# LouisPwr/CarpeDeam

Measured on AMD Instinct MI355X. Metric: corrected bases/sec on 50M×100bp synthetic reads (dhigh), 1/2/4/8 GPU, higher is better.
Workload: dtype u8 (2-bit packed bases; int32 scores; software x87 f80 likelihood sums)

## Files before the change

carpedeam_amd/csrc/aggvote.h:

```cpp
#pragma once
#include "runsort.h"

namespace aggv {

struct Ent { uint32_t id, diag, cs; };
constexpr uint32_t PENDING = 0xFFFFFFFFu;

__global__ __launch_bounds__(1024) void k_seg_flags(const uint32_t *__restrict__ recRep, uint64_t nRec, uint32_t *__restrict__ flag) {
    const uint64_t j = (uint64_t) blockIdx.x * blockDim.x + threadIdx.x;
    if (j <= nRec) flag[j] = (j < nRec && (j == 0 || recRep[j - 1] != recRep[j])) ? 1u : 0u;
}
__global__ __launch_bounds__(1024) void k_seg_fill(const uint32_t *__restrict__ recRep, uint64_t nRec, uint32_t *__restrict__ segOfRec, uint32_t *__restrict__ segRep,
                                                   unsigned long long *__restrict__ segFirstRec, uint32_t *__restrict__ entCnt) {
    const uint64_t j = (uint64_t) blockIdx.x * blockDim.x + threadIdx.x;
    if (j > nRec) return;
    const uint32_t ex = segOfRec[j];
    if (j == nRec) { segFirstRec[ex] = nRec; return; }
    const bool start = j == 0 || recRep[j - 1] != recRep[j];
    const uint32_t g = start ? ex : ex - 1;
    segOfRec[j] = g;
    if (start) { segRep[g] = recRep[j]; segFirstRec[g] = j; entCnt[g] = PENDING; }
}

struct AggArgs {
    const uint64_t *keys; const uint64_t *recVal; const unsigned long long *dst; uint64_t nRec;
    const uint32_t *segOfRec, *segRep; const unsigned long long *segFirstRec; uint64_t nSeg;
    unsigned long long *entOff; uint32_t *entCnt; unsigned long long *perRep;
    Ent *ent; unsigned long long *cursor; unsigned long long cap; unsigned int *overflow;
    int repShift, diagBits; uint32_t idBits;
    uint32_t maxD;
    const uint64_t *sorted;
    const unsigned long long *list; const unsigned int *count;
    bucket::BigList hard;
    unsigned int nextClass = 0;
    int wideWord = 0;
};
constexpr int AG_H = 1024, AG_D = 512, AG_IDX = 9, AG_ORD = 11;
constexpr unsigned long long AG_CHUNK = 2048;
inline unsigned long long aggChunkSlack(unsigned long long units, unsigned long long segments, int cuCount) {
    const unsigned long long g = (unsigned long long) cuCount * 64;
    return (3 * std::min(units + 1, g) + std::min(segments + 1, g)) * AG_CHUNK;
}
static_assert((1 << AG_IDX) >= AG_D && (1 << AG_ORD) > runsort::U_T, "aggregation geometry");
__device__ __forceinline__ uint32_t aggHash(uint64_t k) { return (uint32_t) ((k * 0x9E3779B97F4A7C15ull) >> 40); }

#ifndef CDM_AGG_MINW
#define CDM_AGG_MINW 4
#endif
template <int NT, int ITEMS, typename W = uint64_t>
__global__ __launch_bounds__(NT, CDM_AGG_MINW) void k_unit_agg(AggArgs a) {
    using namespace runsort;
    __shared__ __align__(8) unsigned char sTab[AG_H * 16];
    unsigned long long *tKey = reinterpret_cast<unsigned long long *>(sTab);
    unsigned int *tCnt = reinterpret_cast<unsigned int *>(sTab + AG_H * 8), *tLast = reinterpret_cast<unsigned int *>(sTab + AG_H * 12);
    unsigned int *oFirst = reinterpret_cast<unsigned int *>(sTab), *oEnt = oFirst + (U_T + 2), *oHit = oEnt + (U_T + 2);
    static_assert(3 * (U_T + 2) * 4 <= AG_H * 16, "the directory fits the table's memory");
    __shared__ unsigned long long dKey[AG_D];
    __shared__ unsigned int dCnt[AG_D], dLast[AG_D];
    __shared__ uint16_t sPerm[AG_D];
    __shared__ uint64_t sGStart[NT];
    __shared__ uint32_t sGOff[NT], sGSeg[NT];
    __shared__ unsigned int sDistinct, sOver, sMaxOrd;
    __shared__ unsigned long long sBase, sChunkAt, sChunkEnd;
    const int tid = threadIdx.x, lane = tid & 63, wave = tid >> 6;
    const unsigned int nUnits = *a.count;
    if (tid == 0) { sChunkAt = 0; sChunkEnd = 0; }
    const int lowBits = a.repShift - 1;
    const uint64_t lowMask = (1ull << lowBits) - 1ull;
    for (unsigned int item = blockIdx.x; item < nUnits; item += gridDim.x) {
        const uint64_t base = a.list[3 * (size_t) item];
        const int m = (int) (a.list[3 * (size_t) item + 1] - base);
        const uint64_t rec0 = a.list[3 * (size_t) item + 2];
        const uint32_t g0 = a.segOfRec[rec0];
        for (int i = tid; i < AG_H; i += NT) { tKey[i] = ~0ull; tCnt[i] = 0u; tLast[i] = 0u; }
        if (tid == 0) { sDistinct = 0; sOver = 0; sMaxOrd = 0; }
        __syncthreads();
        const unsigned long long endG = base + (uint64_t) m;
        for (uint64_t c0 = rec0; c0 < a.nRec; c0 += NT) {
            const uint64_t j = c0 + tid;
            const unsigned long long d = j < a.nRec ? a.dst[j] : ~0ull;
            const bool valid = d < endG;
            sGOff[tid] = valid ? (uint32_t) (d - base) : (uint32_t) m;
            sGStart[tid] = valid ? (a.recVal[j] >> RUN_CNT_BITS) : 0ull;
            sGSeg[tid] = valid ? a.segOfRec[j] - g0 : 0u;
            const int nr = __syncthreads_count(valid);
            if (nr == 0) break;
            const int e0 = (int) sGOff[0], e1 = (nr == NT) ? (int) min((unsigned long long) m, (j0Next(a.dst, a.nRec, c0 + NT) - base)) : m;
            if (tid == 0) sMaxOrd = max(sMaxOrd, sGSeg[nr - 1]);
            for (int eb = e0; eb < e1; eb += NT * ITEMS) {
                uint64_t key[ITEMS]; uint32_t ordv[ITEMS];
#pragma unroll
                for (int k = 0; k < ITEMS; k++) {
                    const int e = eb + k * NT + tid;
                    if (e < e1) {
                        int r = 0;
#pragma unroll
                        for (int st = NT / 2; st > 0; st >>= 1) if (r + st < nr && (int) sGOff[r + st] <= e) r += st;
                        key[k] = a.keys[sGStart[r] + (uint64_t) (e - (int) sGOff[r])];
                        ordv[k] = sGSeg[r];
                    }
                }
#pragma unroll
                for (int k = 0; k < ITEMS; k++) {
                    const int e = eb + k * NT + tid;
                    if (e < e1) {
                        const uint64_t hk = ((uint64_t) ordv[k] << lowBits) | ((key[k] >> 1) & lowMask);
                        const unsigned int last = ((unsigned int) e << 1) | (unsigned int) (key[k] & 1ull);
                        uint32_t h = aggHash(hk) & (AG_H - 1);
                        int probe = 0;
                        for (; probe < AG_H; probe++) {
                            unsigned long long old = __hip_atomic_load(&tKey[h], __ATOMIC_RELAXED, __HIP_MEMORY_SCOPE_WORKGROUP);
                            if (old == ~0ull) {
                                old = atomicCAS(&tKey[h], ~0ull, (unsigned long long) hk);
                                if (old == ~0ull) { atomicAdd(&sDistinct, 1u); old = hk; }
                            }
                            if (old == hk) { atomicAdd(&tCnt[h], 1u); atomicMax(&tLast[h], last); break; }
                            h = (h + 1) & (AG_H - 1);
                        }
                        if (probe == AG_H) sOver = 1u;
                    }
                }
            }
            const bool stop = __syncthreads_or(sDistinct > a.maxD || sOver != 0u);
            if (stop || nr < NT) break;
        }
        __syncthreads();
        if (sDistinct > a.maxD || sOver) {
            if (tid == 0) a.hard.add(base, base + (uint64_t) m);
            __syncthreads();
            continue;
        }
        unsigned int c = 0;
        for (int i = tid; i < AG_H; i += NT) c += tKey[i] != ~0ull;
        unsigned int D;
        unsigned int pos = cdm_block_excl_sum<unsigned int>(c, D);
        for (int i = tid; i < AG_H; i += NT) if (tKey[i] != ~0ull) { dKey[pos] = tKey[i]; dCnt[pos] = tCnt[i]; dLast[pos] = tLast[i]; pos++; }
        __syncthreads();
        if (wave == 0) {
            bucket::sortGroup<W>((int) D, lane,
                [&](int i) { return ((W) dKey[i] << AG_IDX) | (W) i; },
                [&](auto &v) {
                    constexpr int R = sizeof(v) / sizeof(v[0]);
#pragma unroll
                    for (int r = 0; r < R; r++) { const int p = lane * R + r; if (p < (int) D) sPerm[p] = (uint16_t) ((uint32_t) v[r] & ((1u << AG_IDX) - 1u)); }
                });
        }
        const unsigned int nOrd = sMaxOrd + 1u;
        for (unsigned int o = tid; o < nOrd; o += NT) { oFirst[o] = 0xFFFFFFFFu; oEnt[o] = 0u; oHit[o] = 0u; }
        if (tid == 0) {
            if (sChunkAt + D > sChunkEnd) { const unsigned long long want = max(AG_CHUNK, (unsigned long long) D); sChunkAt = atomicAdd(a.cursor, want); sChunkEnd = sChunkAt + want; }
            const unsigned long long b = sChunkAt;
            sChunkAt += D;
            if (b + D > a.cap) { atomicExch(a.overflow, 1u); sBase = ~0ull; } else sBase = b;
        }
        __syncthreads();
        const uint64_t idMask = (1ull << a.idBits) - 1ull, diagMask = (1ull << a.diagBits) - 1ull;
        for (unsigned int p = tid; p < D; p += NT) {
            const uint64_t hk = dKey[sPerm[p]], prev = p ? dKey[sPerm[p - 1]] : ~0ull;
            const uint32_t o = (uint32_t) (hk >> lowBits);
            atomicMin(&oFirst[o], p);
            atomicAdd(&oEnt[o], 1u);
            if (p == 0 || (hk >> a.diagBits) != (prev >> a.diagBits)) {
                const uint32_t id = (uint32_t) ((hk >> a.diagBits) & idMask);
                if (id != a.segRep[g0 + o]) atomicAdd(&oHit[o], 1u);
            }
        }
        __syncthreads();
        const unsigned long long b = sBase;
        if (b != ~0ull) {
            for (unsigned int p = tid; p < D; p += NT) {
                const int i = sPerm[p]; const uint64_t hk = dKey[i];
                Ent e; e.id = (uint32_t) ((hk >> a.diagBits) & idMask); e.diag = (uint32_t) (hk & diagMask); e.cs = (dCnt[i] << 1) | (dLast[i] & 1u);
                a.ent[b + p] = e;
            }
            for (unsigned int o = tid; o < nOrd; o += NT) {
                a.entOff[g0 + o] = b + oFirst[o]; a.entCnt[g0 + o] = oEnt[o];
                a.perRep[a.segRep[g0 + o]] = oHit[o];
            }
        }
        __syncthreads();
    }
}

__global__ __launch_bounds__(1024) void k_pending_list(const uint32_t *__restrict__ entCnt, uint64_t nSeg, uint32_t *__restrict__ list, unsigned int *__restrict__ cnt) {
    const uint64_t g = (uint64_t) blockIdx.x * blockDim.x + threadIdx.x;
    const bool p = g < nSeg && entCnt[g] == PENDING;
    const uint32_t q = cdm_block_append(cnt, p);
    if (p) list[q] = (uint32_t) g;
}
__global__ __launch_bounds__(256) void k_rle_segment(AggArgs a, const uint32_t *__restrict__ list, const unsigned int *__restrict__ nList) {
    const unsigned int n = *nList;
    const int lane = threadIdx.x & 63;
    const uint64_t idMask = (1ull << a.idBits) - 1ull, diagMask = (1ull << a.diagBits) - 1ull;
    const uint64_t below = (1ull << lane) - 1ull;
    unsigned long long chunkAt = 0, chunkEnd = 0;
    for (unsigned int it = blockIdx.x * (blockDim.x >> 6) + (threadIdx.x >> 6); it < n; it += gridDim.x * (blockDim.x >> 6)) {
        const uint32_t g = list[it];
        const uint64_t s = a.dst[a.segFirstRec[g]], e = a.dst[a.segFirstRec[g + 1]];
        const uint32_t rep = a.segRep[g];
        unsigned int runs = 0, hits = 0;
        for (uint64_t i = s + lane; i < e; i += 64) {
            const uint64_t k = a.sorted[i], p = i > s ? a.sorted[i - 1] : ~0ull;
            if (i == s || (k >> 1) != (p >> 1)) runs++;
            if (i == s || (k >> (a.diagBits + 1)) != (p >> (a.diagBits + 1))) hits += ((uint32_t) ((k >> (a.diagBits + 1)) & idMask) != rep);
        }
        const unsigned int D = (unsigned int) cdm_wave_sum((int) runs), H = (unsigned int) cdm_wave_sum((int) hits);
        unsigned long long b = 0;
        if (lane == 0) {
            if (chunkAt + D > chunkEnd) { const unsigned long long want = max(AG_CHUNK, (unsigned long long) D); chunkAt = atomicAdd(a.cursor, want); chunkEnd = chunkAt + want; }
            b = chunkAt; chunkAt += D;
            if (b + D > a.cap) { atomicExch(a.overflow, 1u); b = ~0ull; }
            else { a.entOff[g] = b; a.entCnt[g] = D; a.perRep[rep] = H; }
        }
        b = (unsigned long long) __shfl((long long) b, 0, 64);
        if (b == ~0ull) continue;
        unsigned long long run = 0;
        for (uint64_t t0 = s; t0 < e; t0 += 64) {
            const uint64_t i = t0 + lane;
            bool start = false; uint64_t k = 0;
            if (i < e) { k = a.sorted[i]; start = i == s || (k >> 1) != (a.sorted[i - 1] >> 1); }
            const uint64_t m = __ballot(start);
            if (start) {
                const uint64_t later = lane < 63 ? (m >> (lane + 1)) : 0ull;
                uint64_t hi;
                if (later) hi = i + (uint64_t) __ffsll((unsigned long long) later);
                else {
                    uint64_t lo = min(t0 + 63, e - 1); hi = e;
                    while (hi - lo > 1) { const uint64_t mid = lo + ((hi - lo) >> 1); if ((a.sorted[mid] >> 1) == (k >> 1)) lo = mid; else hi = mid; }
                }
                Ent en; en.id = (uint32_t) ((k >> (a.diagBits + 1)) & idMask); en.diag = (uint32_t) ((k >> 1) & diagMask);
                en.cs = ((uint32_t) (hi - i) << 1) | (uint32_t) (a.sorted[hi - 1] & 1ull);
                a.ent[b + run + (unsigned long long) __popcll(m & below)] = en;
            }
            run += (unsigned long long) __popcll(m);
        }
    }
}

struct VoteEntArgs {
    const Ent *ent; const unsigned long long *entOff; const uint32_t *entCnt; const uint32_t *segRep; uint64_t nSeg;
    const uint64_t *hitOff;
    const uint32_t *stale;
    int diagBias;
    const uint32_t *cont = nullptr;
};
constexpr int HEAD_WORDS = 2048;
__global__ void k_head_entries(const Ent *__restrict__ ent, const unsigned long long *__restrict__ entOff, const uint32_t *__restrict__ entCnt, uint64_t nSeg, uint32_t *__restrict__ out) {
    if (nSeg == 0) { out[0] = 0; out[1] = 0; out[2] = 1; out[HEAD_WORDS + 3] = 0; return; }
    const uint32_t id = ent[entOff[0]].id;
    uint32_t words = 0; bool whole = true;
    for (uint64_t g = 0; g < nSeg && whole && words <= (uint32_t) HEAD_WORDS; g++) {
        const Ent *e = ent + entOff[g]; const uint32_t c = entCnt[g];
        for (uint32_t j = 0; j < c; j++) {
            if (e[j].id != id) { whole = false; break; }
            if (words + 2 <= (uint32_t) HEAD_WORDS) { out[3 + words] = e[j].diag | ((e[j].cs & 1u) ? 0u : 1u << 31); out[4 + words] = e[j].cs >> 1; words += 2; }
            else { words = (uint32_t) HEAD_WORDS + 1; whole = false; break; }
        }
    }
    out[0] = words; out[1] = id; out[2] = whole ? 1u : 0u;
    const uint64_t gl = nSeg - 1;
    out[HEAD_WORDS + 3] = ent[entOff[gl] + entCnt[gl] - 1].id;
}
// ... 47 lines not shown
```

carpedeam_amd/csrc/kmermatch.hip:

```cpp
#include <memory>
#include <cstring>

#include "aggvote.h"
#include "kmer_plan.h"
#include "kmer_tuple.h"
#include "kmer_extract.h"
#include "kmer_group.h"
#include "kmer_vote.h"

namespace {

using rx::DoubleBuf;
using namespace kplan;
static_assert(RADIX_BITS == rx::BITS && SLOT_REM_BITS == rx::SLOT_REM, "kmer_plan.h restates the radix sort's geometry");
inline uint64_t deviceBytes() { size_t fr = 0, tot = 0; if (hipMemGetInfo(&fr, &tot) == hipSuccess) return tot; (void) hipGetLastError(); return 0; }
inline Db planDb(const cdm_seqdb *db, int k, bool device = false) { Db d; d.n = db->n; d.maxLen = db->maxLen; d.residues = db->residues; d.k = k; if (device) d.deviceBytes = deviceBytes(); return d; }

struct KmerJobBase {
    virtual ~KmerJobBase() {}
    virtual int phaseA() = 0;
    virtual int staleTail(unsigned long long J) = 0;
    virtual int phaseB(cdm_hits **out) = 0;
    virtual int gatherByRep() = 0;
    virtual int sortFrom(const uint64_t *devKeys, uint64_t nKeys, uint32_t *head, uint64_t info[2]) = 0;
// ... 534 lines not shown
    DoubleBuf<uint32_t> rep; DoubleBuf<uint64_t> val;
};
int recordsByRep(const runsort::RunArgs &ra, bool staged, bool dstIfNone, RepRecords &R, unsigned long long &total) {
    if (staged) { if (int rc = stagedRunRecords(ra, R.r0, R.r1, R.v0, R.v1, R.nRec)) return rc; }
    else if (int rc = runsort::makeRunRecords(s, ra, R.r0, R.r1, R.v0, R.v1, R.nRec)) return rc;
    if (R.nRec == 0 && !dstIfNone) return CDM_OK;
    if (!R.dst.alloc(R.nRec + 1)) { cdm_set_error("cdm_kmermatch: out of device memory (%llu run records)", R.nRec); return CDM_ERR_HIP; }
    if (R.nRec == 0) return CDM_OK;
    R.rep = DoubleBuf<uint32_t>(R.r0.p, R.r1.p); R.val = DoubleBuf<uint64_t>(R.v0.p, R.v1.p);
    if (int rc = rx::sortPairs<uint32_t, uint64_t>(s, ctx->cuCount, R.rep, R.val, (uint64_t) R.nRec, 0, (int) idBits)) return rc;
    hipMemsetAsync(R.val.current() + R.nRec, 0, 8, s);
    if (int rc = cdmscan::exclusiveScanFn<unsigned long long, runsort::RunLen>(s, R.st, runsort::RunLen{R.val.current()}, R.dst.p, (size_t) R.nRec + 1)) return rc;
    hipMemcpyAsync(&total, R.dst.p + R.nRec, 8, hipMemcpyDeviceToHost, s);
    return CDM_OK;
}
int stagedRunRecords(const runsort::RunArgs &whole, DevBuf<uint32_t> &rr0, DevBuf<uint32_t> &rr1, DevBuf<uint64_t> &rv0, DevBuf<uint64_t> &rv1, unsigned long long &nRec) {
    DevBuf<unsigned long long> off; cdmscan::ScanTemp st;
    if (!off.alloc(stagedWaves + 1)) { cdm_set_error("cdm_kmermatch: out of device memory (run records)"); return CDM_ERR_HIP; }
    if (int rc = cdmscan::exclusiveScanFn<unsigned long long, RecCount>(s, st, RecCount{stCnt.p}, off.p, (size_t) stagedWaves + 1)) return rc;
    unsigned long long n1 = 0, n2 = 0;
    hipMemcpyAsync(&n1, off.p + stagedWaves, 8, hipMemcpyDeviceToHost, s);
    DevBuf<uint32_t> q0, q1; DevBuf<uint64_t> w0, w1;
    runsort::RunArgs r2 = whole; r2.keys = whole.keys + kmerSlots; r2.n = whole.n - kmerSlots; r2.skipLo = r2.skipHi = 0; r2.base = kmerSlots;
    if (r2.n) { if (int rc = runsort::makeRunRecords(s, r2, q0, q1, w0, w1, n2)) return rc; }
    if (hipStreamSynchronize(s) != hipSuccess) { cdm_set_error("cdm_kmermatch: run records failed: %s", hipGetErrorString(hipGetLastError())); return CDM_ERR_HIP; }
    unsigned long long nb = nBigRec;
    if (nOvRec) {
        DevBuf<uint64_t> x0, x1; DevBuf<uint32_t> y0, y1;
        const unsigned long long tot = nBigRec + nOvRec;
        if (!x0.alloc(tot) || !x1.alloc(tot) || !y0.alloc(tot) || !y1.alloc(tot)) { cdm_set_error("cdm_kmermatch: out of device memory (run records)"); return CDM_ERR_HIP; }
        if (nBigRec) { hipMemcpyAsync(x0.p, bigRecVal.p, nBigRec * 8, hipMemcpyDeviceToDevice, s); hipMemcpyAsync(y0.p, bigRecRep.p, nBigRec * 4, hipMemcpyDeviceToDevice, s); }
        hipMemcpyAsync(x0.p + nBigRec, ovVal.p, nOvRec * 8, hipMemcpyDeviceToDevice, s); hipMemcpyAsync(y0.p + nBigRec, ovRep.p, nOvRec * 4, hipMemcpyDeviceToDevice, s);
        DoubleBuf<uint64_t> x(x0.p, x1.p); DoubleBuf<uint32_t> y(y0.p, y1.p);
        if (int rc = rx::sortPairs<uint64_t, uint32_t>(s, ctx->cuCount, x, y, (uint64_t) tot, runsort::RUN_CNT_BITS, 64)) return rc;
        bigRecVal.free(); bigRecRep.free();
        bigRecVal.p = x.current() == x0.p ? x0.release() : x1.release(); bigRecRep.p = y.current() == y0.p ? y0.release() : y1.release();
        nb = tot;
    }
    nRec = n1 + nb + n2;
    if (!rr0.alloc(nRec) || !rr1.alloc(nRec) || !rv0.alloc(nRec + 1) || !rv1.alloc(nRec + 1)) { cdm_set_error("cdm_kmermatch: out of device memory (%llu run records)", nRec); return CDM_ERR_HIP; }
    if (n1) hipLaunchKernelGGL(k_rec_compact, CDM_GRID((stagedWaves + REC_WAVES - 1) / REC_WAVES, 256), dim3(256), 0, s, (const uint32_t *) stRep.p, (const uint64_t *) stVal.p, (const unsigned long long *) off.p, (uint64_t) stagedWaves,
                               (uint64_t) stagedOwn, (const uint64_t *) bigRecVal.p, (uint64_t) nb, rr0.p, rv0.p);
    if (nb) hipLaunchKernelGGL(k_rec_place_big, CDM_GRID((nb + 255) / 256, 256), dim3(256), 0, s, (const uint32_t *) bigRecRep.p, (const uint64_t *) bigRecVal.p, (uint64_t) nb, (const uint64_t *) stVal.p, (const uint8_t *) stCnt.p,
                               (const unsigned long long *) off.p, (uint64_t) stagedOwn, rr0.p, rv0.p);
    if (n2) { hipMemcpyAsync(rr0.p + n1 + nb, q0.p, n2 * 4, hipMemcpyDeviceToDevice, s); hipMemcpyAsync(rv0.p + n1 + nb, w0.p, n2 * 8, hipMemcpyDeviceToDevice, s); }
    if (hipStreamSynchronize(s) != hipSuccess) { cdm_set_error("cdm_kmermatch: run records (packing) failed: %s", hipGetErrorString(hipGetLastError())); return CDM_ERR_HIP; }
    if (cdmGetenv("CDM_BUCKET_STATS")) fprintf(stderr, "run records: %llu staged by the grouping kernel, %llu beyond its waves' stages, %llu of its big buckets, %llu of the whole-sequence hash region\n", n1, nOvRec, nBigRec, n2);
    stRep.free(); stVal.free(); stCnt.free(); bigRecRep.free(); bigRecVal.free(); ovRep.free(); ovVal.free(); stagedWaves = 0; nBigRec = 0; nOvRec = 0;
    return CDM_OK;
}
int voteEntries(cdm_hits **out, const uint32_t *contDev = nullptr) {
    DevBuf<unsigned long long> perRepScan;
    if (!perRepScan.alloc((size_t) n + 1)) { cdm_set_error("cdm_kmermatch: out of device memory (vote)"); return CDM_ERR_HIP; }
    cdmscan::ScanTemp st4a;
    if (int rc = cdmscan::exclusiveScan<unsigned long long>(s, st4a, agPerRep.p, perRepScan.p, (size_t) n + 1)) return rc;
    if (int rc = placeHits(perRepScan.p, true, out, [&](cdm_hits *res) {
        aggv::VoteEntArgs va; va.ent = agEnt.p; va.entOff = agEntOff.p; va.entCnt = agEntCnt.p; va.segRep = agSegRep.p; va.nSeg = nSegM; va.hitOff = res->off; va.stale = staleBuf.p; va.diagBias = diagBias; va.cont = contDev;
        if (nSegM) hipLaunchKernelGGL(aggv::k_vote_entries<HitRec>, dim3((unsigned) ((nSegM + 255) / 256)), dim3(256), 0, s, va, res->rec);
    })) return rc;
    agEnt.free(); agEntOff.free(); agEntCnt.free(); agSegRep.free(); agSegOfRec.free(); agSegFirstRec.free(); agPerRep.free(); agPending.free();
    return CDM_OK;
}
template <typename Place>
int placeHits(const unsigned long long *perRepScan, bool sort1R2, cdm_hits **out, Place place) {
    cdm_hits *res = new cdm_hits(); res->n = n;
    if (cdmMalloc(&res->off, ((size_t) n + 1) * 8) != hipSuccess) { delete res; cdm_set_error("cdm_kmermatch: out of device memory"); return CDM_ERR_HIP; }
    hipLaunchKernelGGL(k_offsets, dim3((n + 256) / 256), dim3(256), 0, s, perRepScan, n, res->off);
    uint64_t total = 0;
    hipMemcpyAsync(&total, res->off + n, 8, hipMemcpyDeviceToHost, s);
    { hipError_t e = hipStreamSynchronize(s); if (e != hipSuccess) { cdm_hits_free(res); cdm_set_error("cdm_kmermatch: vote failed: %s", hipGetErrorString(e)); return CDM_ERR_HIP; } }
    res->count = total;
    if (cdmMalloc(&res->rec, (total + 1) * sizeof(HitRec)) != hipSuccess) { cdm_hits_free(res); cdm_set_error("cdm_kmermatch: out of device memory"); return CDM_ERR_HIP; }
    hipLaunchKernelGGL(k_self, dim3((n + 255) / 256), dim3(256), 0, s, res->off, n, res->rec);
    place(res);
    { hipError_t e = hipStreamSynchronize(s); if (e != hipSuccess) { cdm_hits_free(res); cdm_set_error("cdm_kmermatch: placing hits failed: %s", hipGetErrorString(e)); return CDM_ERR_HIP; } }
    float msSort2 = 0; hipEventElapsedTime(&msSort2, ctx->ev0, ctx->ev1);
    ctx->lastMs[2] = msSort1 + msSort2;
    ctx->lastMs[5] = msSort1;
    ctx->lastMs[6] = msSort2;
    if (sort1R2) hipEventElapsedTime(&ctx->lastMs[7], ctx->ev2, ctx->ev3);
    *out = res;
    return CDM_OK;
}
static void aggUnitHook(hipStream_t st, unsigned int grid, const unsigned long long *list, const unsigned int *count, bucket::BigList hard, void *user) {
    aggv::AggArgs *u = reinterpret_cast<aggv::AggArgs *>(user);
    aggv::AggArgs a = *u;
    a.list = list; a.count = count; a.hard = hard;
    const int cls = (int) (u->nextClass++ % runsort::U_CLASSES);
    const unsigned int pad = cdm_lds_pad("CDM_LDS_PAD_AGG");
    if (u->wideWord) {
        if (cls == 0) hipLaunchKernelGGL((aggv::k_unit_agg<256, runsort::U_CLASS_CAP[0] / 256, bucket::u128>), dim3(grid), dim3(256), pad, st, a);
        else if (cls == 1) hipLaunchKernelGGL((aggv::k_unit_agg<256, runsort::U_CLASS_CAP[1] / 256, bucket::u128>), dim3(grid), dim3(256), pad, st, a);
        else hipLaunchKernelGGL((aggv::k_unit_agg<256, runsort::U_CLASS_CAP[2] / 256, bucket::u128>), dim3(grid), dim3(256), pad, st, a);
        return;
    }
    if (cls == 0) hipLaunchKernelGGL((aggv::k_unit_agg<256, runsort::U_CLASS_CAP[0] / 256>), dim3(grid), dim3(256), pad, st, a);
    else if (cls == 1) hipLaunchKernelGGL((aggv::k_unit_agg<256, runsort::U_CLASS_CAP[1] / 256>), dim3(grid), dim3(256), pad, st, a);
    else hipLaunchKernelGGL((aggv::k_unit_agg<256, runsort::U_CLASS_CAP[2] / 256>), dim3(grid), dim3(256), pad, st, a);
}
int aggregate(uint64_t *sortedOut, unsigned long long nGroup, const uint32_t *recRep, const uint64_t *recVal, const unsigned long long *dst, unsigned long long nRec,
              const uint64_t *gk, int top2, unsigned long long capEnt, bool wideWord) {
    using namespace aggv;
    cdmscan::ScanTemp st;
    agEnt.free(); agSegOfRec.free(); agPerRep.free(); agCursor.free(); agFlags.free(); agSegRep.free(); agSegFirstRec.free(); agEntOff.free(); agEntCnt.free(); agPending.free();
    if (!agSegOfRec.alloc(nRec + 2) || !agPerRep.alloc((size_t) n + 1) || !agCursor.alloc(2) || !agFlags.alloc(4)) { cdm_set_error("cdm_kmermatch: out of device memory (aggregation)"); return CDM_ERR_HIP; }
    hipLaunchKernelGGL(k_seg_flags, CDM_GRID((nRec + 1024) / 1024, 1024), dim3(1024), 0, s, recRep, (uint64_t) nRec, agSegOfRec.p);
    if (int rc = cdmscan::exclusiveScan<uint32_t>(s, st, agSegOfRec.p, agSegOfRec.p, (size_t) nRec + 1)) return rc;
    uint32_t nSeg = 0;
    hipMemcpyAsync(&nSeg, agSegOfRec.p + nRec, 4, hipMemcpyDeviceToHost, s);
    if (hipStreamSynchronize(s) != hipSuccess) { cdm_set_error("cdm_kmermatch: aggregation (segments) failed: %s", hipGetErrorString(hipGetLastError())); return CDM_ERR_HIP; }
    if (!agSegRep.alloc(nSeg + 1) || !agSegFirstRec.alloc((size_t) nSeg + 2) || !agEntOff.alloc((size_t) nSeg + 1) || !agEntCnt.alloc((size_t) nSeg + 1) || !agPending.alloc((size_t) nSeg + 1) ||
        !agEnt.alloc(capEnt + 1)) {
        agEnt.free(); cdm_set_error("cdm_kmermatch: out of device memory (aggregation)"); return CDM_ERR_HIP;
    }
    hipLaunchKernelGGL(k_seg_fill, CDM_GRID((nRec + 1024) / 1024, 1024), dim3(1024), 0, s, recRep, (uint64_t) nRec, agSegOfRec.p, agSegRep.p, agSegFirstRec.p, agEntCnt.p);
    hipMemsetAsync(agPerRep.p, 0, ((size_t) n + 1) * 8, s);
    hipMemsetAsync(agCursor.p, 0, 16, s); hipMemsetAsync(agFlags.p, 0, 16, s);
    AggArgs a;
    a.keys = gk; a.recVal = recVal; a.dst = dst; a.nRec = nRec; a.segOfRec = agSegOfRec.p; a.segRep = agSegRep.p; a.segFirstRec = agSegFirstRec.p; a.nSeg = nSeg;
    a.entOff = agEntOff.p; a.entCnt = agEntCnt.p; a.perRep = agPerRep.p; a.ent = agEnt.p; a.cursor = agCursor.p; a.cap = capEnt; a.overflow = agFlags.p;
    a.maxD = AG_D;
    if (const char *e = cdmGetenv("CDM_AGG_D")) { const long v = atol(e); if (v >= 1 && v <= AG_D) a.maxD = (uint32_t) v; }
    a.repShift = (int) (idBits + diagBits + 1); a.diagBits = (int) diagBits; a.idBits = idBits; a.sorted = sortedOut; a.list = nullptr; a.count = nullptr; a.hard.list = nullptr; a.hard.cnt = nullptr;
    a.wideWord = wideWord ? 1 : 0;
    if (runsort::segmentedSortKeys(s, ctx->cuCount, sortedOut, sortedOut, nGroup, (int) (idBits + diagBits + 1), (int) (diagBits + 1), top2, recRep, dst, nRec, gk, recVal, aggUnitHook, &a, wide, agSegOfRec.p, (int) bitsFor((uint64_t) nSeg + 1), agSegFirstRec.p, (uint64_t) nSeg) != CDM_OK) {
        cdm_set_error("cdm_kmermatch: segmented sort 2 failed: %s", hipGetErrorString(hipGetLastError())); return CDM_ERR_HIP;
    }
    hipLaunchKernelGGL(k_pending_list, dim3((unsigned) (((uint64_t) nSeg + 1023) / 1024)), dim3(1024), 0, s, (const uint32_t *) agEntCnt.p, (uint64_t) nSeg, agPending.p, agFlags.p + 1);
    unsigned int fl[4] = {0, 0, 0, 0};
    hipMemcpyAsync(fl, agFlags.p, 16, hipMemcpyDeviceToHost, s);
    if (hipStreamSynchronize(s) != hipSuccess) { cdm_set_error("cdm_kmermatch: aggregation failed: %s", hipGetErrorString(hipGetLastError())); return CDM_ERR_HIP; }
    if (fl[1] && cdmGetenv("CDM_RLE_STATS")) {
        std::vector<uint32_t> pl(fl[1]); std::vector<unsigned long long> fr((size_t) nSeg + 1), dd((size_t) nRec + 1);
        hipMemcpy(pl.data(), agPending.p, (size_t) fl[1] * 4, hipMemcpyDeviceToHost); hipMemcpy(fr.data(), agSegFirstRec.p, ((size_t) nSeg + 1) * 8, hipMemcpyDeviceToHost);
        hipMemcpy(dd.data(), dst, ((size_t) nRec + 1) * 8, hipMemcpyDeviceToHost);
        unsigned long long tot = 0, mx = 0, over4k = 0, over64k = 0, inBig = 0;
        for (uint32_t g : pl) { const unsigned long long m = dd[fr[g + 1]] - dd[fr[g]]; tot += m; mx = std::max(mx, m); if (m > 4096) { over4k++; inBig += m; } if (m > 65536) over64k++; }
        fprintf(stderr, "rle segments: %u of %llu, %llu tuples (longest %llu; %llu beyond 4096 tuples holding %llu, %llu beyond 65536)\n", fl[1], (unsigned long long) nSeg, tot, mx, over4k, inBig, over64k);
    }
    if (fl[1] && !fl[0]) {
        hipLaunchKernelGGL(k_rle_segment, dim3(std::min<unsigned int>((fl[1] + 3) / 4, (unsigned int) ctx->cuCount * 16)), dim3(256), 0, s, a, (const uint32_t *) agPending.p, (const unsigned int *) (agFlags.p + 1));
        hipMemcpyAsync(fl, agFlags.p, 16, hipMemcpyDeviceToHost, s);
        if (hipStreamSynchronize(s) != hipSuccess) { cdm_set_error("cdm_kmermatch: aggregation (segments of the tuple sorters) failed: %s", hipGetErrorString(hipGetLastError())); return CDM_ERR_HIP; }
    }
    unsigned long long used = 0;
    hipMemcpy(&used, agCursor.p, 8, hipMemcpyDeviceToHost);
    if (cdmGetenv("CDM_BUCKET_STATS")) fprintf(stderr, "aggregate: %llu group tuples, %u segments, %llu entries (room for %llu), %u segments through the tuple sorters%s\n", nGroup, nSeg, used, capEnt, fl[1],
                                            fl[0] ? "; entry buffer overflow" : "");
    if (fl[0]) { agEnt.free(); return CDM_ERR_UNSUPPORTED; }
    nSegM = nSeg;
    return CDM_OK;
}
int vote(const uint32_t *contDev, bool ownBuffers, cdm_hits **out) {
    if (haveEntries) return voteEntries(out, contDev);
    const uint64_t *sorted2 = sorted2M; const unsigned long long nGroup = nGroupM;
    DevBuf<unsigned long long> perRep, perRepScan, vTileCnt, vTileOff;
    const uint64_t vTiles = (nGroup + CP_TILE - 1) / CP_TILE;
    if (!perRep.alloc((size_t) n + 1) || !perRepScan.alloc((size_t) n + 1) || !vTileCnt.alloc(vTiles + 1) || !vTileOff.alloc(vTiles + 1)) {
        cdm_set_error("cdm_kmermatch: out of device memory (vote)"); return CDM_ERR_HIP;
    }
    hipMemsetAsync(perRep.p, 0, ((size_t) n + 1) * 8, s);
    hipMemsetAsync(vTileCnt.p, 0, (vTiles + 1) * 8, s);
    VoteArgs va;
    if (ownBuffers && nGroup != nKept) { cdm_set_error("cdm_kmermatch: internal error: %llu group tuples counted, %llu sorted", nKept, nGroup); return CDM_ERR_HIP; }
    va.stale = staleBuf.p; va.cont = contDev;
    va.keys = sorted2; va.n = nGroup; va.idBits = idBits; va.diagBits = diagBits; va.diagBias = diagBias; va.perRep = perRep.p;
    if (nGroup) hipLaunchKernelGGL(k_seg_count, dim3((unsigned) vTiles), dim3(256), 0, s, va, vTileCnt.p);
    cdmscan::ScanTemp st4a, st4b;
    if (int rc = cdmscan::exclusiveScan<unsigned long long>(s, st4a, perRep.p, perRepScan.p, (size_t) n + 1)) return rc;
    if (int rc = cdmscan::exclusiveScan<unsigned long long>(s, st4b, vTileCnt.p, vTileOff.p, (size_t) vTiles + 1)) return rc;
    return placeHits(perRepScan.p, ownBuffers, out, [&](cdm_hits *res) {
        if (nGroup) hipLaunchKernelGGL(k_seg_place, dim3((unsigned) vTiles), dim3(256), cdm_lds_pad("CDM_LDS_PAD_VOTE"), s, va, vTileOff.p, perRepScan.p, res->off, res->rec);
    });
}
int gatherByRep() override {
    using namespace runsort;
    v0.free(); v1.free();
    RunArgs ra; ra.keys = (const uint64_t *) startIo; ra.n = nTuples; ra.skipLo = live; ra.skipHi = kmerSlots; ra.repShift = (int) (idBits + diagBits + 1);
    unsigned long long nOut = 0;
    RepRecords R;
    if (int rc = recordsByRep(ra, stagedWaves != 0, false, R, nOut)) return rc;
    gathered = keys.current();
    if (R.nRec == 0) return CDM_OK;
    hipLaunchKernelGGL(k_run_gather, CDM_GRID((R.nRec + 255) / 256, 256), dim3(256), 0, s, (const uint64_t *) startIo, (const uint64_t *) R.val.current(), (const unsigned long long *) R.dst.p, (uint64_t) R.nRec, gathered);
    if (hipStreamSynchronize(s) != hipSuccess) { cdm_set_error("cdm_kmermatch: gather by representative failed: %s", hipGetErrorString(hipGetLastError())); return CDM_ERR_HIP; }
    if (nOut != nKept) { cdm_set_error("cdm_kmermatch: internal error: %llu group tuples counted, %llu gathered", nKept, nOut); return CDM_ERR_HIP; }
    return CDM_OK;
}
int sortFrom(const uint64_t *devKeys, uint64_t nKeys, uint32_t *head, uint64_t info[2]) override {
    k0.free(); k1.free(); v0.free(); v1.free();
    if (!recvA.alloc(nKeys) || !recvB.alloc(nKeys) || !contBuf.alloc(CONT_CAP + 4)) { cdm_set_error("cdm_kmermatch: out of device memory for %llu received group tuples", (unsigned long long) nKeys); return CDM_ERR_HIP; }
    if (nKeys) hipMemcpyAsync(recvB.p, devKeys, nKeys * 8, hipMemcpyDeviceToDevice, s);
    if (int rc = sort2(recvB.p, nKeys, 0, 0, recvA.p, recvB.p, false)) return rc;
    if (haveEntries) {
        static_assert(aggv::HEAD_WORDS == CONT_CAP, "the words of a head");
        uint32_t lastId = 0;
        hipLaunchKernelGGL(aggv::k_head_entries, dim3(1), dim3(1), 0, s, (const aggv::Ent *) agEnt.p, (const unsigned long long *) agEntOff.p, (const uint32_t *) agEntCnt.p, (uint64_t) nSegM, contBuf.p);
        hipMemcpyAsync(head, contBuf.p, (CONT_CAP + 3) * 4, hipMemcpyDeviceToHost, s);
        hipMemcpyAsync(&lastId, contBuf.p + CONT_CAP + 3, 4, hipMemcpyDeviceToHost, s);
        if (hipStreamSynchronize(s) != hipSuccess) { cdm_set_error("cdm_kmermatch: second half (aggregation) failed: %s", hipGetErrorString(hipGetLastError())); return CDM_ERR_HIP; }
        info[0] = nGroupM; info[1] = lastId;
        return CDM_OK;
    }
    hipLaunchKernelGGL(k_head_segment, dim3(1), dim3(1), 0, s, sorted2M, (uint64_t) nGroupM, idBits, diagBits, contBuf.p);
    uint64_t last = 0;
    hipMemcpyAsync(head, contBuf.p, (CONT_CAP + 3) * 4, hipMemcpyDeviceToHost, s);
    if (nGroupM) hipMemcpyAsync(&last, sorted2M + nGroupM - 1, 8, hipMemcpyDeviceToHost, s);
    if (hipStreamSynchronize(s) != hipSuccess) { cdm_set_error("cdm_kmermatch: second half (sort) failed: %s", hipGetErrorString(hipGetLastError())); return CDM_ERR_HIP; }
    info[0] = nGroupM; info[1] = (last >> (diagBits + 1)) & ((1ull << idBits) - 1ull);
    return CDM_OK;
}
int voteWith(const uint32_t *cont, const uint32_t *staleIn, cdm_hits **out) override {
    if (hipMemcpyAsync(staleBuf.p, staleIn, (STALE_MAX + 3) * 4, hipMemcpyHostToDevice, s) != hipSuccess) { cdm_set_error("cdm_kmermatch: stale list upload failed"); return CDM_ERR_HIP; }
    if (cont) {
// ... 296 lines not shown
```

Before: 17.55 billion.

## Restructure unit aggregation: bitmask record lookup, four-wave split sort, prefetch next unit

The per-unit aggregation kernel now finds each tuple's owning record with an LDS bitmask plus popcount prefix instead of a binary search. Compaction uses insertion indices packed into the high bits of the count, so the block scan goes away. Entries are bucketed by segment ordinal and split across all four waves for sorting, where before only wave 0 sorted. Entry writes are fused into the hit-counting pass. Table clearing moves to the end of each iteration, and the next unit's list and first record batch are prefetched. The cost is more LDS reuse, more code complexity and a new U_CAP limit on unit size, above which units go to the hard path. Optional stats counters and a grid override are also added.

```diff
diff --git a/carpedeam_amd/csrc/aggvote.h b/carpedeam_amd/csrc/aggvote.h
--- a/carpedeam_amd/csrc/aggvote.h
+++ b/carpedeam_amd/csrc/aggvote.h
@@ -33,6 +33,7 @@
     const unsigned long long *list; const unsigned int *count;
     bucket::BigList hard;
     unsigned int nextClass = 0;
+    unsigned int *stats = nullptr; unsigned int cls = 0;
     int wideWord = 0;
 };
 constexpr int AG_H = 1024, AG_D = 512, AG_IDX = 9, AG_ORD = 11;
@@ -44,17 +45,26 @@
 static_assert((1 << AG_IDX) >= AG_D && (1 << AG_ORD) > runsort::U_T, "aggregation geometry");
 __device__ __forceinline__ uint32_t aggHash(uint64_t k) { return (uint32_t) ((k * 0x9E3779B97F4A7C15ull) >> 40); }
 
+enum { ST_CLASS = 0 , ST_ROUNDS = 3, ST_D = 4 , ST_ONEWAVE = 9, ST_ORD = 10 , ST_ORD64 = 13, ST_COLL = 14 , ST_N = 16 };
+constexpr int AG_MASKW = runsort::U_CAP / 64;
+static_assert(runsort::U_CAP % 64 == 0 && AG_MASKW <= 64, "a wave scans the mask's popcounts in one step");
+
+__device__ __forceinline__ uint32_t aggUni(uint32_t v) { return (uint32_t) __builtin_amdgcn_readfirstlane((int) v); }
+__device__ __forceinline__ uint64_t aggUni(uint64_t v) { return ((uint64_t) aggUni((uint32_t) (v >> 32)) << 32) | aggUni((uint32_t) v); }
+
 #ifndef CDM_AGG_MINW
 #define CDM_AGG_MINW 4
 #endif
-template <int NT, int ITEMS, typename W = uint64_t>
+template <int NT, int ITEMS, typename W = uint64_t, bool STATS = false>
 __global__ __launch_bounds__(NT, CDM_AGG_MINW) void k_unit_agg(AggArgs a) {
     using namespace runsort;
+    static_assert(NT == 256 && AG_D % NT == 0, "four waves share the entry sort; a thread ranks AG_D / NT entries");
     __shared__ __align__(8) unsigned char sTab[AG_H * 16];
     unsigned long long *tKey = reinterpret_cast<unsigned long long *>(sTab);
     unsigned int *tCnt = reinterpret_cast<unsigned int *>(sTab + AG_H * 8), *tLast = reinterpret_cast<unsigned int *>(sTab + AG_H * 12);
     unsigned int *oFirst = reinterpret_cast<unsigned int *>(sTab), *oEnt = oFirst + (U_T + 2), *oHit = oEnt + (U_T + 2);
-    static_assert(3 * (U_T + 2) * 4 <= AG_H * 16, "the directory fits the table's memory");
+    unsigned int *sCut = oHit + (U_T + 2);
+    static_assert((3 * (U_T + 2) + 4) * 4 <= AG_H * 16, "the directory fits the table's memory");
     __shared__ unsigned long long dKey[AG_D];
     __shared__ unsigned int dCnt[AG_D], dLast[AG_D];
     __shared__ uint16_t sPerm[AG_D];
@@ -63,42 +73,74 @@
     __shared__ unsigned int sDistinct, sOver, sMaxOrd;
     __shared__ unsigned long long sBase, sChunkAt, sChunkEnd;
     const int tid = threadIdx.x, lane = tid & 63, wave = tid >> 6;
+    unsigned long long *sMask = dKey;
+    unsigned int *sPref = reinterpret_cast<unsigned int *>(dKey + AG_MASKW) + wave * AG_MASKW;
+    uint16_t *sPlace = reinterpret_cast<uint16_t *>(sGStart);
+    static_assert(AG_MASKW * 8 + 4 * AG_MASKW * 4 <= AG_D * 8 && AG_D * 2 <= NT * 8, "mask, popcounts and order fit the memory they borrow");
     const unsigned int nUnits = *a.count;
     if (tid == 0) { sChunkAt = 0; sChunkEnd = 0; }
     const int lowBits = a.repShift - 1;
     const uint64_t lowMask = (1ull << lowBits) - 1ull;
+    for (int i = tid; i < AG_H; i += NT) { tKey[i] = ~0ull; tCnt[i] = 0u; tLast[i] = 0u; }
+    unsigned long long nBase = 0, nEnd = 0, nRec0 = 0; uint64_t pRV = 0; uint32_t pG0 = 0, pSeg = 0, pOff = ~0u, pE1 = 0;
+    auto fetchRecords = [&]() {
+        const uint64_t j = nRec0 + tid;
+        const unsigned long long d = j < a.nRec ? a.dst[j] : ~0ull;
+        pG0 = a.segOfRec[nRec0]; pRV = j < a.nRec ? a.recVal[j] : 0ull; pSeg = j < a.nRec ? a.segOfRec[j] : 0u;
+        pOff = d < nEnd ? (uint32_t) (d - nBase) : ~0u;
+        pE1 = (uint32_t) min(nEnd - nBase, j0Next(a.dst, a.nRec, nRec0 + NT) - nBase);
+    };
+    constexpr bool AHEAD_REC = sizeof(W) == 8;
+    if (blockIdx.x < nUnits) {
+        nBase = a.list[3 * (size_t) blockIdx.x]; nEnd = a.list[3 * (size_t) blockIdx.x + 1]; nRec0 = a.list[3 * (size_t) blockIdx.x + 2];
+        if (AHEAD_REC) fetchRecords();
+    }
     for (unsigned int item = blockIdx.x; item < nUnits; item += gridDim.x) {
-        const uint64_t base = a.list[3 * (size_t) item];
-        const int m = (int) (a.list[3 * (size_t) item + 1] - base);
-        const uint64_t rec0 = a.list[3 * (size_t) item + 2];
-        const uint32_t g0 = a.segOfRec[rec0];
-        for (int i = tid; i < AG_H; i += NT) { tKey[i] = ~0ull; tCnt[i] = 0u; tLast[i] = 0u; }
+        if (!AHEAD_REC) fetchRecords();
+        const uint64_t base = aggUni((uint64_t) nBase);
+        const int m = (int) aggUni((uint32_t) (nEnd - nBase));
+        const uint64_t rec0 = aggUni((uint64_t) nRec0);
+        const uint32_t g0 = aggUni(pG0), seg0 = pSeg, off0 = pOff, e1p = pE1;
+        const uint64_t rv0 = pRV;
+        const bool hasNext = item + gridDim.x < nUnits;
+        if (hasNext) { const size_t q = 3 * (size_t) (item + gridDim.x); nBase = a.list[q]; nEnd = a.list[q + 1]; nRec0 = a.list[q + 2]; }
+        const bool fits = m <= U_CAP;
+        if (tid < AG_MASKW) sMask[tid] = 0ull;
         if (tid == 0) { sDistinct = 0; sOver = 0; sMaxOrd = 0; }
         __syncthreads();
         const unsigned long long endG = base + (uint64_t) m;
-        for (uint64_t c0 = rec0; c0 < a.nRec; c0 += NT) {
+        int rounds = 0;
+        for (uint64_t c0 = rec0; fits; c0 += NT) {
             const uint64_t j = c0 + tid;
-            const unsigned long long d = j < a.nRec ? a.dst[j] : ~0ull;
-            const bool valid = d < endG;
-            sGOff[tid] = valid ? (uint32_t) (d - base) : (uint32_t) m;
-            sGStart[tid] = valid ? (a.recVal[j] >> RUN_CNT_BITS) : 0ull;
-            sGSeg[tid] = valid ? a.segOfRec[j] - g0 : 0u;
+            const bool first = c0 == rec0;
+            const unsigned long long d = first ? 0ull : j < a.nRec ? a.dst[j] : ~0ull;
+            const bool valid = first ? off0 != ~0u : d < endG;
+            const uint32_t off = valid ? (first ? off0 : (uint32_t) (d - base)) : (uint32_t) m;
+            sGOff[tid] = off;
+            sGStart[tid] = valid ? ((first ? rv0 : a.recVal[j]) >> RUN_CNT_BITS) : 0ull;
+            sGSeg[tid] = valid ? (first ? seg0 : a.segOfRec[j]) - g0 : 0u;
+            if (valid && off < (uint32_t) U_CAP) atomicOr(&sMask[off >> 6], 1ull << (off & 63u));
             const int nr = __syncthreads_count(valid);
             if (nr == 0) break;
-            const int e0 = (int) sGOff[0], e1 = (nr == NT) ? (int) min((unsigned long long) m, (j0Next(a.dst, a.nRec, c0 + NT) - base)) : m;
+            if (STATS) rounds++;
+            {
+                const unsigned int c = lane < AG_MASKW ? (unsigned int) __popcll(sMask[lane]) : 0u;
+                const unsigned int incl = cdm_wave_incl_sum<unsigned int>(c);
+                if (lane < AG_MASKW) sPref[lane] = incl - c;
+                if (STATS && tid == AG_MASKW - 1 && incl != (unsigned int) nr) atomicAdd(&a.stats[ST_COLL], 1u);
+                bucket::waveLdsSync();
+            }
+            const int e0 = (int) sGOff[0], e1 = (nr == NT) ? (first ? (int) e1p : (int) min((unsigned long long) m, j0Next(a.dst, a.nRec, c0 + NT) - base)) : m;
             if (tid == 0) sMaxOrd = max(sMaxOrd, sGSeg[nr - 1]);
             for (int eb = e0; eb < e1; eb += NT * ITEMS) {
                 uint64_t key[ITEMS]; uint32_t ordv[ITEMS];
 #pragma unroll
                 for (int k = 0; k < ITEMS; k++) {
-                    const int e = eb + k * NT + tid;
-                    if (e < e1) {
-                        int r = 0;
-#pragma unroll
-                        for (int st = NT / 2; st > 0; st >>= 1) if (r + st < nr && (int) sGOff[r + st] <= e) r += st;
-                        key[k] = a.keys[sGStart[r] + (uint64_t) (e - (int) sGOff[r])];
-                        ordv[k] = sGSeg[r];
-                    }
+                    const int e = min(eb + k * NT + tid, e1 - 1);
+                    const int wd = e >> 6;
+                    const int r = min(max((int) sPref[wd] + __popcll(sMask[wd] & ((2ull << (e & 63)) - 1ull)) - 1, 0), NT - 1);
+                    key[k] = a.keys[sGStart[r] + (uint64_t) (e - (int) sGOff[r])];
+                    ordv[k] = sGSeg[r];
                 }
 #pragma unroll
                 for (int k = 0; k < ITEMS; k++) {
@@ -110,11 +152,12 @@
                         int probe = 0;
                         for (; probe < AG_H; probe++) {
                             unsigned long long old = __hip_atomic_load(&tKey[h], __ATOMIC_RELAXED, __HIP_MEMORY_SCOPE_WORKGROUP);
+                            unsigned int add = 1u;
                             if (old == ~0ull) {
                                 old = atomicCAS(&tKey[h], ~0ull, (unsigned long long) hk);
-                                if (old == ~0ull) { atomicAdd(&sDistinct, 1u); old = hk; }
+                                if (old == ~0ull) { const unsigned int ix = atomicAdd(&sDistinct, 1u); if (ix < (unsigned int) AG_D) add += ix << 16; old = hk; }
                             }
-                            if (old == hk) { atomicAdd(&tCnt[h], 1u); atomicMax(&tLast[h], last); break; }
+                            if (old == hk) { atomicAdd(&tCnt[h], add); atomicMax(&tLast[h], last); break; }
                             h = (h + 1) & (AG_H - 1);
                         }
                         if (probe == AG_H) sOver = 1u;
@@ -123,30 +166,32 @@
             }
             const bool stop = __syncthreads_or(sDistinct > a.maxD || sOver != 0u);
             if (stop || nr < NT) break;
-        }
-        __syncthreads();
-        if (sDistinct > a.maxD || sOver) {
+            if (tid < AG_MASKW) sMask[tid] = 0ull;
+            __syncthreads();
+        }
+        __syncthreads();
+        if (AHEAD_REC && hasNext) fetchRecords();
+        if (STATS && tid == 0) { atomicAdd(&a.stats[ST_CLASS + a.cls], 1u); if (rounds > 1) atomicAdd(&a.stats[ST_ROUNDS], 1u); }
+        if (!fits || sDistinct > a.maxD || sOver) {
             if (tid == 0) a.hard.add(base, base + (uint64_t) m);
+            if (STATS && tid == 0) atomicAdd(&a.stats[ST_D + 4], 1u);
+            for (int i = tid; i < AG_H; i += NT) { tKey[i] = ~0ull; tCnt[i] = 0u; tLast[i] = 0u; }
             __syncthreads();
             continue;
         }
-        unsigned int c = 0;
-        for (int i = tid; i < AG_H; i += NT) c += tKey[i] != ~0ull;
-        unsigned int D;
-        unsigned int pos = cdm_block_excl_sum<unsigned int>(c, D);
-        for (int i = tid; i < AG_H; i += NT) if (tKey[i] != ~0ull) { dKey[pos] = tKey[i]; dCnt[pos] = tCnt[i]; dLast[pos] = tLast[i]; pos++; }
-        __syncthreads();
-        if (wave == 0) {
-            bucket::sortGroup<W>((int) D, lane,
-                [&](int i) { return ((W) dKey[i] << AG_IDX) | (W) i; },
-                [&](auto &v) {
-                    constexpr int R = sizeof(v) / sizeof(v[0]);
-#pragma unroll
-                    for (int r = 0; r < R; r++) { const int p = lane * R + r; if (p < (int) D) sPerm[p] = (uint16_t) ((uint32_t) v[r] & ((1u << AG_IDX) - 1u)); }
-                });
-        }
-        const unsigned int nOrd = sMaxOrd + 1u;
-        for (unsigned int o = tid; o < nOrd; o += NT) { oFirst[o] = 0xFFFFFFFFu; oEnt[o] = 0u; oHit[o] = 0u; }
+        const unsigned int D = aggUni(sDistinct);
+        for (int i = tid; i < AG_H; i += NT) {
+            const unsigned long long k = tKey[i];
+            if (k != ~0ull) {
+                const unsigned int cw = tCnt[i], pos = cw >> 16;
+                dKey[pos] = k; dCnt[pos] = cw & 0xFFFFu; dLast[pos] = tLast[i];
+                tKey[i] = ~0ull; tCnt[i] = 0u; tLast[i] = 0u;
+            }
+        }
+        __syncthreads();
+        const unsigned int nOrd = aggUni(sMaxOrd) + 1u;
+        for (unsigned int o = tid; o < nOrd; o += NT) { oEnt[o] = 0u; oHit[o] = 0u; }
+        if (tid < 4) sCut[tid] = tid ? D : 0u;
         if (tid == 0) {
             if (sChunkAt + D > sChunkEnd) { const unsigned long long want = max(AG_CHUNK, (unsigned long long) D); sChunkAt = atomicAdd(a.cursor, want); sChunkEnd = sChunkAt + want; }
             const unsigned long long b = sChunkAt;
@@ -154,30 +199,70 @@
             if (b + D > a.cap) { atomicExch(a.overflow, 1u); sBase = ~0ull; } else sBase = b;
         }
         __syncthreads();
+        uint32_t eOrd[AG_D / NT], eRank[AG_D / NT];
+#pragma unroll
+        for (int k = 0; k < AG_D / NT; k++) {
+            const unsigned int p = (unsigned int) (tid + k * NT);
+            if (p < D) { eOrd[k] = (uint32_t) (dKey[p] >> lowBits); eRank[k] = atomicAdd(&oEnt[eOrd[k]], 1u); }
+        }
+        __syncthreads();
+        unsigned int carry = 0;
+        for (unsigned int o0 = 0; o0 < nOrd; o0 += 64) {
+            const unsigned int o = o0 + (unsigned int) lane;
+            const unsigned int n = o < nOrd ? oEnt[o] : 0u;
+            const unsigned int incl = cdm_wave_incl_sum<unsigned int>(n);
+            const unsigned int f = carry + incl - n;
+            if (o < nOrd) {
+                oFirst[o] = f;
+                if (n) { const unsigned int w = f * 4u / D; for (unsigned int q = 1; q <= w; q++) atomicMin(&sCut[q], f); }
+            }
+            carry += (unsigned int) __shfl((int) incl, 63, 64);
+        }
+        bucket::waveLdsSync();
+#pragma unroll
+        for (int k = 0; k < AG_D / NT; k++) {
+            const unsigned int p = (unsigned int) (tid + k * NT);
+            if (p < D) sPlace[oFirst[eOrd[k]] + eRank[k]] = (uint16_t) p;
+        }
+        __syncthreads();
+        const unsigned int s0 = aggUni(sCut[wave]), s1 = wave < 3 ? aggUni(sCut[wave + 1]) : D;
+        bucket::sortGroup<W>((int) (s1 - s0), lane,
+            [&](int i) { const unsigned int q = sPlace[s0 + (unsigned int) i]; return ((W) dKey[q] << AG_IDX) | (W) q; },
+            [&](auto &v) {
+                constexpr int R = sizeof(v) / sizeof(v[0]);
+#pragma unroll
+                for (int r = 0; r < R; r++) { const unsigned int p = (unsigned int) (lane * R + r); if (p < s1 - s0) sPerm[s0 + p] = (uint16_t) ((uint32_t) v[r] & ((1u << AG_IDX) - 1u)); }
+            });
+        bucket::waveLdsSync();
         const uint64_t idMask = (1ull << a.idBits) - 1ull, diagMask = (1ull << a.diagBits) - 1ull;
-        for (unsigned int p = tid; p < D; p += NT) {
-            const uint64_t hk = dKey[sPerm[p]], prev = p ? dKey[sPerm[p - 1]] : ~0ull;
-            const uint32_t o = (uint32_t) (hk >> lowBits);
-            atomicMin(&oFirst[o], p);
-            atomicAdd(&oEnt[o], 1u);
-            if (p == 0 || (hk >> a.diagBits) != (prev >> a.diagBits)) {
-                const uint32_t id = (uint32_t) ((hk >> a.diagBits) & idMask);
+        const unsigned long long b = sBase;
+        for (unsigned int p = s0 + (unsigned int) lane; p < s1; p += 64) {
+            const int i = sPerm[p];
+            const uint64_t hk = dKey[i], prev = p > s0 ? dKey[sPerm[p - 1]] : ~0ull;
+            const uint32_t id = (uint32_t) ((hk >> a.diagBits) & idMask);
+            if (p == s0 || (hk >> a.diagBits) != (prev >> a.diagBits)) {
+                const uint32_t o = (uint32_t) (hk >> lowBits);
                 if (id != a.segRep[g0 + o]) atomicAdd(&oHit[o], 1u);
             }
-        }
-        __syncthreads();
-        const unsigned long long b = sBase;
+            if (b != ~0ull) { Ent e; e.id = id; e.diag = (uint32_t) (hk & diagMask); e.cs = (dCnt[i] << 1) | (dLast[i] & 1u); a.ent[b + p] = e; }
+        }
+        if (STATS && tid == 0) {
+            atomicAdd(&a.stats[ST_D + (D <= 64 ? 0 : D <= 128 ? 1 : D <= 256 ? 2 : 3)], 1u);
+            if (sCut[1] == D) atomicAdd(&a.stats[ST_ONEWAVE], 1u);
+            atomicAdd(&a.stats[ST_ORD + (nOrd == 1 ? 0 : nOrd <= 4 ? 1 : 2)], 1u);
+            if (nOrd > 64) atomicAdd(&a.stats[ST_ORD64], 1u);
+        }
+        __syncthreads();
         if (b != ~0ull) {
-            for (unsigned int p = tid; p < D; p += NT) {
-                const int i = sPerm[p]; const uint64_t hk = dKey[i];
-                Ent e; e.id = (uint32_t) ((hk >> a.diagBits) & idMask); e.diag = (uint32_t) (hk & diagMask); e.cs = (dCnt[i] << 1) | (dLast[i] & 1u);
-                a.ent[b + p] = e;
-            }
             for (unsigned int o = tid; o < nOrd; o += NT) {
                 a.entOff[g0 + o] = b + oFirst[o]; a.entCnt[g0 + o] = oEnt[o];
                 a.perRep[a.segRep[g0 + o]] = oHit[o];
             }
         }
+        for (unsigned int o = tid; o < nOrd; o += NT) {
+            oFirst[o] = 0xFFFFFFFFu; oEnt[o] = (U_T + 2) + o < 2u * AG_H ? 0xFFFFFFFFu : 0u; oHit[o] = 0u;
+        }
+        if (tid < 4) sCut[tid] = 0u;
         __syncthreads();
     }
 }
diff --git a/carpedeam_amd/csrc/kmermatch.hip b/carpedeam_amd/csrc/kmermatch.hip
--- a/carpedeam_amd/csrc/kmermatch.hip
+++ b/carpedeam_amd/csrc/kmermatch.hip
@@ -640,21 +640,23 @@
     *out = res;
     return CDM_OK;
 }
+template <typename W, bool STATS>
+static void aggLaunch(hipStream_t st, int cls, unsigned int grid, unsigned int pad, const aggv::AggArgs &a) {
+    if (cls == 0) hipLaunchKernelGGL((aggv::k_unit_agg<256, runsort::U_CLASS_CAP[0] / 256, W, STATS>), dim3(grid), dim3(256), pad, st, a);
+    else if (cls == 1) hipLaunchKernelGGL((aggv::k_unit_agg<256, runsort::U_CLASS_CAP[1] / 256, W, STATS>), dim3(grid), dim3(256), pad, st, a);
+    else hipLaunchKernelGGL((aggv::k_unit_agg<256, runsort::U_CLASS_CAP[2] / 256, W, STATS>), dim3(grid), dim3(256), pad, st, a);
+}
 static void aggUnitHook(hipStream_t st, unsigned int grid, const unsigned long long *list, const unsigned int *count, bucket::BigList hard, void *user) {
     aggv::AggArgs *u = reinterpret_cast<aggv::AggArgs *>(user);
     aggv::AggArgs a = *u;
     a.list = list; a.count = count; a.hard = hard;
     const int cls = (int) (u->nextClass++ % runsort::U_CLASSES);
+    a.cls = (unsigned int) cls;
     const unsigned int pad = cdm_lds_pad("CDM_LDS_PAD_AGG");
-    if (u->wideWord) {
-        if (cls == 0) hipLaunchKernelGGL((aggv::k_unit_agg<256, runsort::U_CLASS_CAP[0] / 256, bucket::u128>), dim3(grid), dim3(256), pad, st, a);
-        else if (cls == 1) hipLaunchKernelGGL((aggv::k_unit_agg<256, runsort::U_CLASS_CAP[1] / 256, bucket::u128>), dim3(grid), dim3(256), pad, st, a);
-        else hipLaunchKernelGGL((aggv::k_unit_agg<256, runsort::U_CLASS_CAP[2] / 256, bucket::u128>), dim3(grid), dim3(256), pad, st, a);
-        return;
-    }
-    if (cls == 0) hipLaunchKernelGGL((aggv::k_unit_agg<256, runsort::U_CLASS_CAP[0] / 256>), dim3(grid), dim3(256), pad, st, a);
-    else if (cls == 1) hipLaunchKernelGGL((aggv::k_unit_agg<256, runsort::U_CLASS_CAP[1] / 256>), dim3(grid), dim3(256), pad, st, a);
-    else hipLaunchKernelGGL((aggv::k_unit_agg<256, runsort::U_CLASS_CAP[2] / 256>), dim3(grid), dim3(256), pad, st, a);
+    if (const char *e = cdmGetenv("CDM_AGG_GRID")) { const long v = atol(e); if (v >= 1) grid = (unsigned int) std::min<long>(v, (long) grid); }
+    if (u->wideWord) { if (a.stats) aggLaunch<bucket::u128, true>(st, cls, grid, pad, a); else aggLaunch<bucket::u128, false>(st, cls, grid, pad, a); }
+    else if (a.stats) aggLaunch<uint64_t, true>(st, cls, grid, pad, a);
+    else aggLaunch<uint64_t, false>(st, cls, grid, pad, a);
 }
 int aggregate(uint64_t *sortedOut, unsigned long long nGroup, const uint32_t *recRep, const uint64_t *recVal, const unsigned long long *dst, unsigned long long nRec,
               const uint64_t *gk, int top2, unsigned long long capEnt, bool wideWord) {
@@ -681,6 +683,12 @@
     if (const char *e = cdmGetenv("CDM_AGG_D")) { const long v = atol(e); if (v >= 1 && v <= AG_D) a.maxD = (uint32_t) v; }
     a.repShift = (int) (idBits + diagBits + 1); a.diagBits = (int) diagBits; a.idBits = idBits; a.sorted = sortedOut; a.list = nullptr; a.count = nullptr; a.hard.list = nullptr; a.hard.cnt = nullptr;
     a.wideWord = wideWord ? 1 : 0;
+    DevBuf<unsigned int> agStats;
+    if (cdmGetenv("CDM_AGG_STATS")) {
+        if (!agStats.alloc(ST_N)) { cdm_set_error("cdm_kmermatch: out of device memory (aggregation)"); return CDM_ERR_HIP; }
+        hipMemsetAsync(agStats.p, 0, ST_N * 4, s);
+        a.stats = agStats.p;
+    }
     if (runsort::segmentedSortKeys(s, ctx->cuCount, sortedOut, sortedOut, nGroup, (int) (idBits + diagBits + 1), (int) (diagBits + 1), top2, recRep, dst, nRec, gk, recVal, aggUnitHook, &a, wide, agSegOfRec.p, (int) bitsFor((uint64_t) nSeg + 1), agSegFirstRec.p, (uint64_t) nSeg) != CDM_OK) {
         cdm_set_error("cdm_kmermatch: segmented sort 2 failed: %s", hipGetErrorString(hipGetLastError())); return CDM_ERR_HIP;
     }
@@ -688,6 +696,12 @@
     unsigned int fl[4] = {0, 0, 0, 0};
     hipMemcpyAsync(fl, agFlags.p, 16, hipMemcpyDeviceToHost, s);
     if (hipStreamSynchronize(s) != hipSuccess) { cdm_set_error("cdm_kmermatch: aggregation failed: %s", hipGetErrorString(hipGetLastError())); return CDM_ERR_HIP; }
+    if (a.stats) {
+        unsigned int t[ST_N];
+        hipMemcpy(t, agStats.p, sizeof t, hipMemcpyDeviceToHost);
+        fprintf(stderr, "k_unit_agg: classes %u %u %u rounds>1 %u D<=64 %u D<=128 %u D<=256 %u D<=512 %u bailed %u onewave %u ord1 %u ord2-4 %u ord>4 %u ord>64 %u collisions %u overflow %u\n",
+                t[ST_CLASS], t[ST_CLASS + 1], t[ST_CLASS + 2], t[ST_ROUNDS], t[ST_D], t[ST_D + 1], t[ST_D + 2], t[ST_D + 3], t[ST_D + 4], t[ST_ONEWAVE], t[ST_ORD], t[ST_ORD + 1], t[ST_ORD + 2], t[ST_ORD64], t[ST_COLL], fl[0]);
+    }
     if (fl[1] && cdmGetenv("CDM_RLE_STATS")) {
         std::vector<uint32_t> pl(fl[1]); std::vector<unsigned long long> fr((size_t) nSeg + 1), dd((size_t) nRec + 1);
         hipMemcpy(pl.data(), agPending.p, (size_t) fl[1] * 4, hipMemcpyDeviceToHost); hipMemcpy(fr.data(), agSegFirstRec.p, ((size_t) nSeg + 1) * 8, hipMemcpyDeviceToHost);
```

Measured after the change: 17.71 billion, median of 6. About the same (+0.9%).
